# irvingzhang0512/tf_eager_object_detection

Measured on AMD Instinct MI355X. Metric: images/sec, higher is better.
Workload: dtype f32

## Files before the change

### tf_eager_object_detection_amd/csrc/nms.hip

```cpp
#include <stddef.h>
#include <string.h>

#include <algorithm>
#include <mutex>

#include "conv_diag.h"

#define NMS_CHUNK 4096
#define NMS_SEL_MAX (2 * NMS_CHUNK)
#define NMS_WORDS (NMS_CHUNK / 64)
#define SEL_BINS 4096
#define SEL_REPL 8
#define SEL_BLOCK 256
#define SEL_ITEMS 8
#define SEL_TILE (SEL_BLOCK * SEL_ITEMS)
#define PREP_ITEMS 2
#define PREP_TILE (256 * PREP_ITEMS)

typedef unsigned long long u64;

#define SCAN_LDS_BLOCKS 24
#define SCAN_LDS_CAND (SCAN_LDS_BLOCKS * 64)
#define SCAN_LDS_WORDS (SCAN_LDS_BLOCKS * (SCAN_LDS_BLOCKS - 1) / 2 * 64)
#define SCAN_LDS_SLACK_WORDS (8 * 64)
#define SCAN_DYN_LDS ((SCAN_LDS_WORDS + SCAN_LDS_SLACK_WORDS) * 8)
#define SCAN_MAT_OFF(cb, nblk) (64 * ((cb) * ((nblk)-1) - (cb) * ((cb)-1) / 2))

struct NmsState {
  int32_t n_invalid;
  int32_t kept;
  int32_t pos;
  int32_t done;
  int32_t chunk_m;
  int32_t sel_count;
  int32_t reserved0;
  int32_t sel_b1;
  uint32_t sel_below1;
  int32_t sel_b2;
  int32_t sel_overflow;
  uint32_t sel_below;
  int32_t pad[4];
};

#define SEL_COARSE 64
struct NmsHeader {
  NmsState st;
  int32_t n_invalid_acc;
  int32_t pad_acc[15];
  uint32_t hist0[SEL_REPL][SEL_COARSE];
  uint32_t hist1[SEL_REPL][SEL_BINS];
  uint32_t hist2[SEL_BINS];
  uint32_t hist3[256];
};

enum { PREP_NMS = 0, PREP_RP = 1, PREP_FPN = 2, PREP_FRCNN = 3 };

struct PrepParams {
  int n;
  PerImg<const float4*> boxes_in;
  PerImg<const float*> deltas;
  PerImg<const float*> scores;
  PerImg<const float2*> logits;
  Vec4 means, stds;
  float wmax, hmax;
  PerImg<float4*> boxes_out;
  PerImg<uint32_t*> keys;
  PerImg<NmsHeader*> hdr;
  FpnAnchorParams fpn;
};

__global__ void __launch_bounds__(256) k_zero_headers(PerImg<NmsHeader*> hdr_) {
  uint4* d = reinterpret_cast<uint4*>(hdr_.v[blockIdx.y]);
  const int i = blockIdx.x * 256 + threadIdx.x;
  if (i < (int)(sizeof(NmsHeader) / 16)) d[i] = make_uint4(0, 0, 0, 0);
}

template <int MODE>
__device__ __forceinline__ float4 d_prep_box(const PrepParams& p, int img, int e) {
  if (MODE == PREP_NMS) return p.boxes_in.v[img][e];
  float4 a;
  if (MODE == PREP_FPN) {
    a = d_fpn_anchor(p.fpn, e);
  } else if (MODE == PREP_FRCNN) {
    const int ai = e % p.fpn.A, cell = e / p.fpn.A;
    const int x = cell % p.fpn.fw[0], y = cell / p.fpn.fw[0];
    const float sx = (float)(x * p.fpn.stride[0]), sy = (float)(y * p.fpn.stride[0]);
    a = make_float4(p.fpn.wh[ai * 4 + 0] + sx, p.fpn.wh[ai * 4 + 1] + sy, p.fpn.wh[ai * 4 + 2] + sx,
                    p.fpn.wh[ai * 4 + 3] + sy);
  } else {
    a = p.boxes_in.v[img][e];
  }
  const float4 d = reinterpret_cast<const float4*>(p.deltas.v[img])[e];
  const float d0 = d.x * p.stds.v[0] + p.means.v[0];
  const float d1 = d.y * p.stds.v[1] + p.means.v[1];
  const float d2 = d.z * p.stds.v[2] + p.means.v[2];
  const float d3 = d.w * p.stds.v[3] + p.means.v[3];
  float4 b = d_decode_box(a, d0, d1, d2, d3);
  return d_clip_box(b, 0.0f, p.wmax, p.hmax);
}

__device__ __forceinline__ float4 d_candidate_box(const PrepParams& p, int mode, int img, int e) {
  switch (mode) {
    case PREP_NMS: return d_prep_box<PREP_NMS>(p, img, e);
    case PREP_RP: return d_prep_box<PREP_RP>(p, img, e);
    case PREP_FRCNN: return d_prep_box<PREP_FRCNN>(p, img, e);
    default: return d_prep_box<PREP_FPN>(p, img, e);
  }
}

struct PrepItems {
  float sc[PREP_ITEMS];
  float2 lg[PREP_ITEMS];
};

template <int MODE>
__device__ __forceinline__ void d_prep_load(const PrepParams& p, const float* __restrict__ in_scores,
                                            const float2* __restrict__ in_logits, int tile, PrepItems* v) {
#pragma unroll
  for (int it = 0; it < PREP_ITEMS; ++it) {
    const int e = tile * PREP_TILE + it * 256 + threadIdx.x;
    const int ee = e < p.n ? e : 0;
    if (MODE == PREP_FPN) {
      v->lg[it] = in_logits[ee];
    } else if (MODE == PREP_FRCNN) {
      const int loc = ee / p.fpn.A, a = ee - loc * p.fpn.A;
      const float* row = reinterpret_cast<const float*>(in_logits) + (size_t)loc * 2 * p.fpn.A;
      v->lg[it] = make_float2(row[a], row[p.fpn.A + a]);
    } else {
      v->sc[it] = in_scores[ee];
    }
  }
}

__device__ __forceinline__ uint32_t d_row16_sum(uint32_t v) {
  v += (uint32_t)__builtin_amdgcn_update_dpp(0, (int)v, 0xB1, 0xF, 0xF, false);
  v += (uint32_t)__builtin_amdgcn_update_dpp(0, (int)v, 0x4E, 0xF, 0xF, false);
  v += (uint32_t)__builtin_amdgcn_update_dpp(0, (int)v, 0x141, 0xF, 0xF, false);
  v += (uint32_t)__builtin_amdgcn_update_dpp(0, (int)v, 0x140, 0xF, 0xF, false);
  return v;
}

template <int MODE, int T>
__global__ void __launch_bounds__(256) k_rp_prepare(PrepParams p) {
  const int img = blockIdx.y;
  const float* __restrict__ in_scores = p.scores.v[img];
  const float2* __restrict__ in_logits = p.logits.v[img];
  uint32_t* __restrict__ out_keys = p.keys.v[img];
  NmsHeader* hdr = p.hdr.v[img];
  __shared__ __attribute__((aligned(16))) uint32_t h[SEL_BINS];
  uint4* h4 = reinterpret_cast<uint4*>(h);
#pragma unroll
  for (int q = 0; q < SEL_BINS / 4 / 256; ++q) h4[q * 256 + threadIdx.x] = make_uint4(0, 0, 0, 0);
  PrepItems cur;
  d_prep_load<MODE>(p, in_scores, in_logits, blockIdx.x * T, &cur);
  __syncthreads();
  int invalid = 0;
#pragma unroll
  for (int t = 0; t < T; ++t) {
    const int tile = blockIdx.x * T + t;
    PrepItems nxt;
    if (t + 1 < T) d_prep_load<MODE>(p, in_scores, in_logits, tile + 1, &nxt);
#pragma unroll
    for (int it = 0; it < PREP_ITEMS; ++it) {
      const int e = tile * PREP_TILE + it * 256 + threadIdx.x;
      if (e < p.n) {
        float s;
        if (MODE == PREP_FPN || MODE == PREP_FRCNN) s = d_fg_prob(cur.lg[it].x, cur.lg[it].y);
        else s = cur.sc[it];
        const bool valid = s > -3.402823466e+38f;
        const uint32_t k = valid ? ~d_float_asc_key(s) : 0xFFFFFFFFu;
        out_keys[e] = k;
        invalid += valid ? 0 : 1;
        atomicAdd(&h[k >> 20], 1u);
      }
    }
    if (t + 1 < T) cur = nxt;
  }
  __syncthreads();
  const int repl = blockIdx.x % SEL_REPL;
  const int lane = threadIdx.x & 63;
#pragma unroll
  for (int q = 0; q < SEL_BINS / 4 / 256; ++q) {
    const int k4 = q * 256 + threadIdx.x;
    const uint4 c = h4[k4];
    uint32_t s = c.x + c.y + c.z + c.w;
    if (__ballot(s != 0)) {
      const int first = (k4 - lane) * 4;
#pragma unroll
      for (int i = 0; i < 4; ++i) {
        const uint32_t v = h[first + i * 64 + lane];
        if (v) atomicAdd(&hdr->hist1[repl][first + i * 64 + lane], v);
      }
    }
    s = d_row16_sum(s);
    if ((threadIdx.x & 15) == 0 && s) atomicAdd(&hdr->hist0[repl][k4 >> 4], s);
  }
  if (invalid) atomicAdd(&hdr->n_invalid_acc, invalid);
}

template <int REPL>
__device__ __forceinline__ void sel_find(const uint32_t* __restrict__ hist, uint32_t target, uint32_t* result,
                                         int* lds17) {
  uint32_t v[16];
#pragma unroll
  for (int q = 0; q < 16; ++q) v[q] = 0;
#pragma unroll
  for (int r = 0; r < REPL; ++r) {
    const uint4* h4 = reinterpret_cast<const uint4*>(hist + (size_t)r * SEL_BINS) + threadIdx.x * 4;
#pragma unroll
    for (int q = 0; q < 4; ++q) {
      const uint4 t = h4[q];
      v[q * 4 + 0] += t.x; v[q * 4 + 1] += t.y; v[q * 4 + 2] += t.z; v[q * 4 + 3] += t.w;
    }
  }
  uint32_t s = 0;
#pragma unroll
  for (int q = 0; q < 16; ++q) s += v[q];
  int total;
  const uint32_t excl = (uint32_t)block_excl_scan((int)s, lds17, &total);
  if ((uint32_t)total < target) target = (uint32_t)total;
  if (threadIdx.x == 0 && total == 0) { result[0] = SEL_BINS - 1; result[1] = 0; result[2] = 0; }
  if (s > 0 && excl < target && target <= excl + s) {
    uint32_t run = excl;
#pragma unroll
    for (int q = 0; q < 16; ++q) {
      if (run < target && target <= run + v[q]) {
        result[0] = threadIdx.x * 16 + q; result[1] = run; result[2] = v[q];
      }
      run += v[q];
    }
  }
  __syncthreads();
}

__device__ __forceinline__ void sel_find1_coarse(const NmsHeader* hdr, uint32_t target, uint32_t* res) {
  if (threadIdx.x < 64) {
    const int t = threadIdx.x;
    int c = 0;
#pragma unroll
    for (int r = 0; r < SEL_REPL; ++r) c += (int)hdr->hist0[r][t];
    const int inc = wave_incl_scan(c);
    const int total = __shfl(inc, 63);
    if (total == 0) {
      if (t == 0) { res[0] = SEL_BINS - 1; res[1] = 0; }
    } else {
      const int tgt = (int)(target > (uint32_t)total ? (uint32_t)total : target);
      const u64 hitc = __ballot(c > 0 && inc - c < tgt && tgt <= inc);
      const int cb = __builtin_ctzll(hitc);
      const int below_c = __shfl(inc - c, cb);
      int v = 0;
#pragma unroll
      for (int r = 0; r < SEL_REPL; ++r) v += (int)hdr->hist1[r][cb * 64 + t];
      const int inc2 = wave_incl_scan(v);
      const u64 hitf = __ballot(v > 0 && below_c + inc2 - v < tgt && tgt <= below_c + inc2);
      const int fb = __builtin_ctzll(hitf);
      const int below_f = __shfl(inc2 - v, fb);
      if (t == 0) { res[0] = (uint32_t)(cb * 64 + fb); res[1] = (uint32_t)(below_c + below_f); }
    }
  }
  __syncthreads();
}

__global__ void __launch_bounds__(SEL_BLOCK) k_sel_hist2(PerImg<NmsHeader*> hdr_, PerImg<const uint32_t*> keys_, int n,
                                                         uint32_t target) {
  NmsHeader* hdr = hdr_.v[blockIdx.y];
  const uint32_t* __restrict__ keys = keys_.v[blockIdx.y];
  __shared__ uint32_t h[SEL_BINS];
  __shared__ uint32_t res[2];
  uint32_t key[SEL_ITEMS];
#pragma unroll
  for (int it = 0; it < SEL_ITEMS; ++it) {
    const int e = blockIdx.x * SEL_TILE + it * SEL_BLOCK + threadIdx.x;
    key[it] = (e < n) ? keys[e] : 0u;
  }
  sel_find1_coarse(hdr, target, res);
  const uint32_t b1 = res[0];
  if (blockIdx.x == 0 && threadIdx.x == 0) {
    NmsState z;
    memset(&z, 0, sizeof(z));
    z.n_invalid = hdr->n_invalid_acc;
    z.sel_b1 = (int32_t)b1; z.sel_below1 = res[1];
    hdr->st = z;
    hdr->n_invalid_acc = 0;
  }
  bool match = false;
#pragma unroll
  for (int it = 0; it < SEL_ITEMS; ++it) {
    const int e = blockIdx.x * SEL_TILE + it * SEL_BLOCK + threadIdx.x;
    match = match || (e < n && (key[it] >> 20) == b1);
  }
  if (!__syncthreads_or(match ? 1 : 0)) return;
  for (int k = threadIdx.x; k < SEL_BINS; k += SEL_BLOCK) h[k] = 0;
  __syncthreads();
#pragma unroll
  for (int it = 0; it < SEL_ITEMS; ++it) {
    const int e = blockIdx.x * SEL_TILE + it * SEL_BLOCK + threadIdx.x;
    if (e < n && (key[it] >> 20) == b1) atomicAdd(&h[(key[it] >> 8) & 0xFFFu], 1u);
  }
  __syncthreads();
  for (int k = threadIdx.x; k < SEL_BINS; k += SEL_BLOCK) {
    const uint32_t c = h[k];
    if (c) atomicAdd(&hdr->hist2[k], c);
  }
}

__global__ void __launch_bounds__(SEL_BLOCK) k_sel_compact(PerImg<NmsHeader*> hdr_, PerImg<const uint32_t*> keys_, int n,
                                                           uint32_t target, uint32_t limit, PerImg<u64*> cand_) {
  NmsHeader* hdr = hdr_.v[blockIdx.y];
  const uint32_t* __restrict__ keys = keys_.v[blockIdx.y];
  u64* __restrict__ cand = cand_.v[blockIdx.y];
  __shared__ uint32_t res[3];
  __shared__ int lds17[17];
  const uint32_t b1 = (uint32_t)hdr->st.sel_b1;
  const uint32_t below1 = hdr->st.sel_below1;
  {
    static_assert(offsetof(NmsHeader, hist1) == offsetof(NmsHeader, hist0) + sizeof(uint32_t) * SEL_REPL * SEL_COARSE, "layout");
    uint4* z = reinterpret_cast<uint4*>(&hdr->hist0[0][0]);
    for (int i = blockIdx.x * SEL_BLOCK + threadIdx.x; i < SEL_REPL * (SEL_COARSE + SEL_BINS) / 4; i += gridDim.x * SEL_BLOCK)
      z[i] = make_uint4(0, 0, 0, 0);
  }
  uint32_t total_n = (uint32_t)n;
  uint32_t t2 = (target > total_n ? total_n : target) - below1;
  sel_find<1>(hdr->hist2, t2, res, lds17);
  const uint32_t b2 = res[0];
  const bool incl = (below1 + res[1] + res[2]) <= limit;
  if (blockIdx.x == 0 && threadIdx.x == 0) {
    hdr->st.sel_b2 = (int32_t)b2;
    hdr->st.sel_overflow = incl ? 0 : 1;
    hdr->st.sel_below = below1 + res[1];
  }
  __shared__ u64 stage[SEL_TILE];
  __shared__ int s_cnt, s_base;
  if (threadIdx.x == 0) s_cnt = 0;
  uint32_t key[SEL_ITEMS];
#pragma unroll
  for (int it = 0; it < SEL_ITEMS; ++it) {
    const int e = blockIdx.x * SEL_TILE + it * SEL_BLOCK + threadIdx.x;
    key[it] = (e < n) ? keys[e] : 0xFFFFFFFFu;
  }
  __syncthreads();
  const int lane = threadIdx.x & 63;
  const u64 lt_mask = (lane == 0) ? 0ull : (~0ull >> (64 - lane));
#pragma unroll
  for (int it = 0; it < SEL_ITEMS; ++it) {
    const int e = blockIdx.x * SEL_TILE + it * SEL_BLOCK + threadIdx.x;
    const uint32_t k = key[it];
    const uint32_t p1 = k >> 20, p2 = (k >> 8) & 0xFFFu;
    const bool sel = (e < n) && (p1 < b1 || (p1 == b1 && (p2 < b2 || (incl && p2 == b2))));
    const u64 bal = __ballot(sel);
    if (bal) {
      int base = 0;
      if (lane == __builtin_ctzll(bal)) base = atomicAdd(&s_cnt, (int)__popcll(bal));
      base = __shfl(base, __builtin_ctzll(bal));
      if (sel) stage[base + (int)__popcll(bal & lt_mask)] = ((u64)k << 32) | (uint32_t)e;
    }
  }
  __syncthreads();
  const int c = s_cnt;
  if (c == 0) return;
  if (threadIdx.x == 0) s_base = atomicAdd(&hdr->st.sel_count, c);
  __syncthreads();
  const int gb = s_base;
  for (int i = threadIdx.x; i < c; i += SEL_BLOCK)
    if (gb + i < NMS_SEL_MAX) cand[gb + i] = stage[i];
}

__global__ void __launch_bounds__(SEL_BLOCK) k_sel_tie_hist(PerImg<NmsHeader*> hdr_, PerImg<const uint32_t*> keys_, int n,
                                                            PerImg<unsigned short*> bh_) {
  NmsHeader* hdr = hdr_.v[blockIdx.y];
  if (!hdr->st.sel_overflow) return;
  const uint32_t* __restrict__ keys = keys_.v[blockIdx.y];
  unsigned short* __restrict__ bh = bh_.v[blockIdx.y] + (size_t)blockIdx.x * 256;
  __shared__ uint32_t h[256];
  const uint32_t pref = ((uint32_t)hdr->st.sel_b1 << 12) | (uint32_t)hdr->st.sel_b2;
  h[threadIdx.x] = 0;
  __syncthreads();
#pragma unroll
  for (int it = 0; it < SEL_ITEMS; ++it) {
    const int e = blockIdx.x * SEL_TILE + it * SEL_BLOCK + threadIdx.x;
    if (e < n) {
      const uint32_t k = keys[e];
      if ((k >> 8) == pref) atomicAdd(&h[k & 0xFFu], 1u);
    }
  }
  __syncthreads();
  const uint32_t c = h[threadIdx.x];
  bh[threadIdx.x] = (unsigned short)c;
  if (c) atomicAdd(&hdr->hist3[threadIdx.x], c);
}

__global__ void __launch_bounds__(SEL_BLOCK) k_sel_tie_take(PerImg<NmsHeader*> hdr_, PerImg<const uint32_t*> keys_, int n,
                                                            uint32_t limit, PerImg<const unsigned short*> bh_,
                                                            PerImg<u64*> cand_) {
  NmsHeader* hdr = hdr_.v[blockIdx.y];
  if (!hdr->st.sel_overflow) return;
  const uint32_t below = hdr->st.sel_below;
  if (below >= limit) return;
  const uint32_t quota = limit - below;
  const uint32_t* __restrict__ keys = keys_.v[blockIdx.y];
  const unsigned short* __restrict__ bh = bh_.v[blockIdx.y];
  u64* __restrict__ cand = cand_.v[blockIdx.y];
  __shared__ int lds17[17];
  __shared__ uint32_t s_b3, s_q3, s_pre;
  __shared__ int s_wave[4];
  __shared__ u64 stage[SEL_TILE];
  __shared__ int s_cnt, s_base;
  const uint32_t pref = ((uint32_t)hdr->st.sel_b1 << 12) | (uint32_t)hdr->st.sel_b2;
  const uint32_t hv = hdr->hist3[threadIdx.x];
  int total;
  const uint32_t excl = (uint32_t)block_excl_scan((int)hv, lds17, &total);
  if (threadIdx.x == 0) { s_b3 = 256; s_q3 = 0; s_pre = 0; s_cnt = 0; }
  __syncthreads();
  if (hv > 0 && excl < quota && quota <= excl + hv) { s_b3 = threadIdx.x; s_q3 = quota - excl; }
  __syncthreads();
  const uint32_t b3 = s_b3, q3 = s_q3;
  if (b3 < 256) {
    uint32_t mine = 0;
    for (int b = threadIdx.x; b < (int)blockIdx.x; b += SEL_BLOCK) mine += bh[(size_t)b * 256 + b3];
    int tot2;
    block_excl_scan((int)mine, lds17, &tot2);
    if (threadIdx.x == 0) s_pre = (uint32_t)tot2;
  }
  __syncthreads();
  uint32_t run = s_pre;
  const int lane = threadIdx.x & 63, wv = threadIdx.x >> 6;
  const u64 lt_mask = (lane == 0) ? 0ull : (~0ull >> (64 - lane));
  for (int it = 0; it < SEL_ITEMS; ++it) {
    const int e = blockIdx.x * SEL_TILE + it * SEL_BLOCK + threadIdx.x;
    const uint32_t k = (e < n) ? keys[e] : 0xFFFFFFFFu;
    const bool inbin = (e < n) && (k >> 8) == pref;
    const uint32_t v = k & 0xFFu;
    const bool tie = inbin && v == b3;
    const u64 tb = __ballot(tie);
    if (lane == 0) s_wave[wv] = (int)__popcll(tb);
    __syncthreads();
    uint32_t before = run;
    for (int q = 0; q < wv; ++q) before += (uint32_t)s_wave[q];
    const uint32_t my_rank = before + (uint32_t)__popcll(tb & lt_mask);
    const uint32_t all4 = (uint32_t)(s_wave[0] + s_wave[1] + s_wave[2] + s_wave[3]);
    const bool sel = inbin && (v < b3 || (tie && my_rank < q3));
    const u64 bal = __ballot(sel);
    if (bal) {
      int base = 0;
      if (lane == __builtin_ctzll(bal)) base = atomicAdd(&s_cnt, (int)__popcll(bal));
      base = __shfl(base, __builtin_ctzll(bal));
      if (sel) stage[base + (int)__popcll(bal & lt_mask)] = ((u64)k << 32) | (uint32_t)e;
    }
    run += all4;
    __syncthreads();
  }
  const int c = s_cnt;
  if (c == 0) return;
  if (threadIdx.x == 0) s_base = atomicAdd(&hdr->st.sel_count, c);
  __syncthreads();
  const int gb = s_base;
  for (int i = threadIdx.x; i < c; i += SEL_BLOCK)
    if (gb + i < NMS_SEL_MAX) cand[gb + i] = stage[i];
}

#define RANK_THREADS 1024
__global__ void __launch_bounds__(RANK_THREADS) k_sel_rank(PerImg<NmsHeader*> hdr_, int n, int cap0, PerImg<const u64*> cand_,
                                                          PrepParams prep, int mode, PerImg<uint32_t*> sel_idx_,
                                                          PerImg<float4*> sboxes_, PerImg<float4*> sorig_) {
  NmsHeader* hdr = hdr_.v[blockIdx.y];
  const u64* __restrict__ cand = cand_.v[blockIdx.y];
  uint32_t* __restrict__ sel_idx = sel_idx_.v[blockIdx.y];
  float4* __restrict__ sboxes = sboxes_.v[blockIdx.y];
  float4* __restrict__ sorig = sorig_.v[blockIdx.y];
  __shared__ u64 all[NMS_CHUNK];
  __shared__ int part[16][64];
  NmsState* st = &hdr->st;
  const int cnt = min(st->sel_count, NMS_SEL_MAX);
  if (blockIdx.x == 0 && threadIdx.x == 0) st->chunk_m = min(min(cnt, cap0), n - st->n_invalid);
  if (blockIdx.x == 0) {
    uint4* z = reinterpret_cast<uint4*>(hdr->hist2);
    for (int i = threadIdx.x; i < SEL_BINS / 4; i += RANK_THREADS) z[i] = make_uint4(0, 0, 0, 0);
    if (threadIdx.x < 256) hdr->hist3[threadIdx.x] = 0;
  }
  if (blockIdx.x * 64 >= cnt) return;
  const int lane = threadIdx.x & 63, w = threadIdx.x >> 6;
  const int i = blockIdx.x * 64 + lane;
  const u64 mine = (i < cnt) ? cand[i] : ~0ull;
  float4 bx = make_float4(0.0f, 0.0f, 0.0f, 0.0f);
  if (w == 0 && i < cnt) bx = d_candidate_box(prep, mode, blockIdx.y, (int)(uint32_t)mine);
  int c = 0;
  for (int t0 = 0; t0 < cnt; t0 += NMS_CHUNK) {
    const int tc = min(NMS_CHUNK, cnt - t0);
    __syncthreads();
    for (int k = threadIdx.x; k < tc; k += RANK_THREADS) all[k] = cand[t0 + k];
    __syncthreads();
    const int per = (tc + 15) >> 4;
    const int lo = w * per, hi = min(tc, lo + per);
    for (int j = lo; j < hi; ++j) c += (all[j] < mine) ? 1 : 0;
  }
  part[w][lane] = c;
  __syncthreads();
  if (w == 0 && i < cnt) {
    int r = 0;
#pragma unroll
    for (int k = 0; k < 16; ++k) r += part[k][lane];
    const uint32_t idx = (uint32_t)mine;
    sel_idx[r] = idx;
    if (r < cap0) {
      sboxes[r] = d_norm_box(bx);
      sorig[r] = bx;
    }
  }
}

__global__ void __launch_bounds__(256) k_nms_gather(PerImg<NmsState*> st_, int n, int cap, int from_sel,
                                                    PrepParams prep, int mode, PerImg<const uint32_t*> sorted_idx_,
                                                    PerImg<float4*> sboxes_, PerImg<float4*> sorig_) {
  NmsState* st = st_.v[blockIdx.y];
  const uint32_t* __restrict__ sorted_idx = sorted_idx_.v[blockIdx.y];
  float4* __restrict__ sboxes = sboxes_.v[blockIdx.y];
  float4* __restrict__ sorig = sorig_.v[blockIdx.y];
  const int pos = st->pos, nv = n - st->n_invalid;
  const int lim = from_sel ? min(nv, min(st->sel_count, NMS_SEL_MAX)) : nv;
  const int m = st->done ? 0 : max(0, min(cap, lim - pos));
  const int i = blockIdx.x * 256 + threadIdx.x;
  if (i == 0) st->chunk_m = m;
  if (i < m) {
    const float4 bx = d_candidate_box(prep, mode, blockIdx.y, (int)sorted_idx[pos + i]);
    sboxes[i] = d_norm_box(bx);
    sorig[i] = bx;
  }
}

__global__ void __launch_bounds__(256) k_nms_cross(PerImg<const NmsState*> st_, PerImg<const float4*> sboxes_,
                                                   PerImg<const float4*> kept_boxes_, float thr,
                                                   PerImg<u64*> removed_init_) {
  const NmsState* st = st_.v[blockIdx.y];
  const float4* __restrict__ sboxes = sboxes_.v[blockIdx.y];
  const float4* __restrict__ kept_boxes = kept_boxes_.v[blockIdx.y];
  u64* __restrict__ removed_init = removed_init_.v[blockIdx.y];
  __shared__ float4 kb[256];
  __shared__ float ka[256];
  const int m = st->chunk_m, nk = st->kept;
  if (blockIdx.x * 256 >= m) return;
  const int j = blockIdx.x * 256 + threadIdx.x;
  const float4 b = (j < m) ? sboxes[j] : make_float4(0, 0, 0, 0);
  const float area = d_box_area(b);
  bool sup = false;
  for (int k0 = 0; k0 < nk; k0 += 256) {
    __syncthreads();
    if (k0 + threadIdx.x < nk) {
      float4 t = kept_boxes[k0 + threadIdx.x];
      kb[threadIdx.x] = t;
      ka[threadIdx.x] = d_box_area(t);
    }
    __syncthreads();
    const int lim = min(256, nk - k0);
    for (int k = 0; k < lim; ++k) sup = sup || d_iou_gt(b, area, kb[k], ka[k], thr);
  }
  u64 bal = __ballot(sup && j < m);
  if ((threadIdx.x & 63) == 0) removed_init[j >> 6] = bal;
}

__global__ void __launch_bounds__(256) k_nms_mask(PerImg<const NmsState*> st_, PerImg<const float4*> sboxes_, float thr,
                                                  PerImg<u64*> Lt_, PerImg<u64*> diag_, int packed) {
// ... 459 lines not shown
          const int l = olvl ? min(max(olvl[r], 0), nlo - 1) : 0;
          int qy, qx;
          bkt[e] = d_roi_order_bucket(osrc[r], l, sp.ord_inv_h, sp.ord_inv_w, &qy, &qx);
          slot[e] = atomicAdd(&ocnt[bkt[e]], 1);
        } else if (r < K) {
          order[r] = r;
        }
      }
      __syncthreads();
      scan_order_buckets(ocnt, nb, keptpre);
      __syncthreads();
#pragma unroll
      for (int e = 0; e < 2; ++e)
        if (bkt[e] >= 0) order[ocnt[bkt[e]] + slot[e]] = tid + e * SCAN_THREADS;
    } else {
      if (tid < K) order[tid] = tid;
      if (tid + SCAN_THREADS < K) order[tid + SCAN_THREADS] = tid + SCAN_THREADS;
    }
  }
}

struct NmsWorkspace {
  NmsHeader* hdr;
  uint32_t *keys_a, *vals_a, *keys_b, *vals_b, *hist;
  u64* cand;
  float4 *sboxes, *sorig, *kept_boxes;
  u64 *Lt, *diag, *removed_init;
};

static size_t nms_carve(int n, int max_out, void* ws, size_t ws_bytes, NmsWorkspace* o) {
  OdetArena ar{(char*)ws, ws ? ws_bytes : (size_t)-1, 0};
  size_t nn = (size_t)(n > 0 ? n : 1);
  size_t kk = (size_t)(max_out > 0 ? max_out : 1);
#define TAKE(field, T, count)                                 \
  do {                                                        \
    T* p_ = ar.take<T>(count);                                \
    if (o) o->field = ws ? p_ : nullptr;                      \
  } while (0)
  TAKE(hdr, NmsHeader, 1);
  TAKE(keys_a, uint32_t, nn);
  TAKE(vals_a, uint32_t, nn);
  TAKE(keys_b, uint32_t, nn);
  TAKE(vals_b, uint32_t, std::max(nn, (size_t)NMS_SEL_MAX));
  TAKE(hist, uint32_t, odet_sort_hist_entries(n));
  TAKE(cand, u64, NMS_SEL_MAX);
  TAKE(sboxes, float4, NMS_CHUNK);
  TAKE(sorig, float4, NMS_CHUNK);
  TAKE(kept_boxes, float4, kk);
  TAKE(Lt, u64, (size_t)NMS_WORDS * NMS_CHUNK);
  TAKE(diag, u64, NMS_CHUNK);
  TAKE(removed_init, u64, NMS_WORDS);
#undef TAKE
  return ar.off + 256;
}

extern "C" size_t odet_nms_workspace_bytes(int n, int max_output) {
  return nms_carve(n, max_output, nullptr, 0, nullptr);
}

static int first_chunk_target(int n, int K, int first_chunk) {
  long long c = ((long long)K * 3 / 2 + 63) / 64 * 64;
  if (c > 64) c -= 32;
  if (first_chunk > 0) c = std::max<long long>(c, ((long long)first_chunk + 63) / 64 * 64 - 32);
  if (c < 256) c = 256;
  if (c > NMS_CHUNK) c = NMS_CHUNK;
  if (c > n) c = n;
  return (int)c;
}

static inline int tri_tiles(int cap) {
  int nb = (cap + 63) / 64;
  return nb * (nb + 1) / 2;
}

struct NmsPlan {
  int n, K, first_chunk, B, sync_free;
  int blind;
  int target;
  int lds0, limit;
  int wide;
  int sel_target, sel_limit;
  int prep_grid, sel_grid, rank_wgs;
  int prep_tiles;
  int cap0, tiles0;
  int cap, tiles;
  int further;
  int sel_chunks;
  int full_sort;
  int fail_empty_chunk;
  int max_chunks;
};

#define PREP_RESIDENT_WGS 2048
#define PREP_MAX_TILES 4
static int nms_prep_tiles(int prep_grid, int B) {
  for (int t = 1; t < PREP_MAX_TILES; t *= 2)
    if ((long long)((prep_grid + t - 1) / t) * B <= PREP_RESIDENT_WGS) return t;
  return PREP_MAX_TILES;
}

static int nms_plan(int n, int K, int first_chunk, int blind_chunks, int sync_free, int B, NmsPlan* out) {
  NmsPlan p;
  p.n = n; p.K = K; p.first_chunk = first_chunk; p.B = B; p.sync_free = sync_free ? 1 : 0;
  p.blind = blind_chunks < 1 ? 1 : blind_chunks;
  p.target = first_chunk_target(n, K, first_chunk);
  p.lds0 = p.target <= SCAN_LDS_CAND ? 1 : 0;
  p.limit = p.lds0 ? SCAN_LDS_CAND : NMS_CHUNK;
  p.wide = (p.sync_free && p.blind >= 2) ? 1 : 0;
  p.sel_target = p.wide ? (int)std::min<long long>(n, (long long)p.target + NMS_CHUNK) : p.target;
  p.sel_limit = p.wide ? NMS_SEL_MAX : p.limit;
  p.prep_grid = (n + PREP_TILE - 1) / PREP_TILE;
  p.prep_tiles = nms_prep_tiles(p.prep_grid, B);
  p.sel_grid = (n + SEL_TILE - 1) / SEL_TILE;
  if (p.wide)
    ODET_REQUIRE((size_t)p.sel_grid * 256 * sizeof(unsigned short) <= (size_t)NMS_WORDS * NMS_CHUNK * sizeof(u64),
                 "odet_nms: %d anchors exceed the tie split's scratch (the bit-matrix buffer)", n);
  p.rank_wgs = (std::min(n, p.sel_limit) + 63) / 64;
  p.cap0 = std::min(p.limit, (n + 63) / 64 * 64);
  p.tiles0 = tri_tiles(p.cap0);
  p.cap = std::min(NMS_CHUNK, (n + 63) / 64 * 64);
  p.tiles = tri_tiles(p.cap);
  p.further = p.sync_free ? p.blind - 1 : 0;
  p.sel_chunks = p.further >= 1 ? 1 : 0;
  p.full_sort = p.further >= 2 ? 1 : 0;
  p.fail_empty_chunk = p.sync_free ? p.blind - 1 : -1;
  p.max_chunks = p.sync_free ? 0 : (n + NMS_CHUNK - 1) / NMS_CHUNK + 1;
  *out = p;
  return ODET_OK;
}

#ifdef ODET_DIAG
static std::mutex g_nms_plan_mutex;
static odet_debug_nms_plan_t g_last_nms_plan;
static void nms_plan_to_record(const NmsPlan& p, odet_debug_nms_plan_t* r, long long count) {
  *r = odet_debug_nms_plan_t{p.n, p.K, p.first_chunk, p.B, p.sync_free, p.blind, p.target, p.lds0, p.limit, p.wide,
                             p.sel_target, p.sel_limit, p.prep_grid, p.sel_grid, p.rank_wgs, p.cap0, p.tiles0, p.cap,
                             p.tiles, p.further, p.sel_chunks, p.full_sort, p.fail_empty_chunk, p.max_chunks, count};
}
static void nms_diag_record(const NmsPlan& p) {
  std::lock_guard<std::mutex> lock(g_nms_plan_mutex);
  nms_plan_to_record(p, &g_last_nms_plan, g_last_nms_plan.count + 1);
}
extern "C" int odet_debug_last_nms_plan(odet_debug_nms_plan_t* out) {
  ODET_REQUIRE(out, "odet_debug_last_nms_plan: null record");
  std::lock_guard<std::mutex> lock(g_nms_plan_mutex);
  *out = g_last_nms_plan;
  return ODET_OK;
}
extern "C" int odet_debug_nms_plan(int n, int K, int first_chunk, int blind_chunks, int sync_free, int B,
                                   odet_debug_nms_plan_t* out) {
  ODET_REQUIRE(out && n > 0 && K > 0 && first_chunk >= 0 && first_chunk <= NMS_CHUNK && B >= 1 && B <= ODET_MAX_BATCH &&
               (sync_free || B == 1), "odet_debug_nms_plan: bad arguments");
  NmsPlan p;
  const int rc = nms_plan(n, K, first_chunk, blind_chunks, sync_free, B, &p);
  if (rc == ODET_OK) nms_plan_to_record(p, out, 0);
  return rc;
}
#define ODET_DIAG_NMS_PLAN(plan)               \
  do {                                         \
    nms_diag_record(plan);                     \
    if (odet_diag_plan_only()) return ODET_OK; \
  } while (0)
#define ODET_DIAG_NMS_TRIVIAL()                \
  do {                                         \
    if (odet_diag_plan_only()) return ODET_OK; \
  } while (0)
#else
#define ODET_DIAG_NMS_PLAN(plan) \
  do {                           \
  } while (0)
#define ODET_DIAG_NMS_TRIVIAL() \
  do {                          \
  } while (0)
#endif

struct NmsImage {
  const float4* boxes_in;
  const float* deltas;
  const float* scores;
  const float2* logits;
  float4* boxes_out;
  const float4* boxes;
  int32_t* out_idx;
  float* out_boxes;
  int32_t* out_count;
  int32_t* out_done;
  AssignOut assign;
  void* ws;
  size_t ws_bytes;
};

struct NmsJob {
  int mode;
  PrepParams prep;
  int n, K;
  float thr;
// ... 37 lines not shown
  else if (J.mode == PREP_FRCNN) nms_prepare_launch<PREP_FRCNN>(J, P, st);
  else nms_prepare_launch<PREP_FPN>(J, P, st);
  ODET_LAUNCH_CHECK();
  return ODET_OK;
}

struct NmsChunks {
  const NmsJob& J;
  const NmsPlan& P;
  hipStream_t st;
  ScanParams sp;
  PerImg<const NmsState*> cstates;
  PerImg<float4*> sboxes, sorig;
  PerImg<const float4*> csboxes, kept;
  PerImg<u64*> Lt, diag, rinit;

  int launch(int from_sel, const PerImg<const uint32_t*>& sorted_idx, int fail_empty) const {
    const dim3 rows((P.cap + 255) / 256, P.B), block(256);
    hipLaunchKernelGGL(k_nms_gather, rows, block, 0, st, sp.st, P.n, P.cap, from_sel, J.prep, J.mode, sorted_idx, sboxes, sorig);
    ODET_LAUNCH_CHECK();
    hipLaunchKernelGGL(k_nms_cross, rows, block, 0, st, cstates, csboxes, kept, J.thr, rinit);
    ODET_LAUNCH_CHECK();
    hipLaunchKernelGGL(k_nms_mask, dim3(P.tiles, P.B), block, 0, st, cstates, csboxes, J.thr, Lt, diag, 0);
    ODET_LAUNCH_CHECK();
    ScanParams s = sp;
    s.use_init = 1; s.sorted_idx = sorted_idx; s.fail_empty = fail_empty;
    hipLaunchKernelGGL(HIP_KERNEL_NAME(k_nms_scan<false>), dim3(1, P.B), dim3(SCAN_THREADS), scan_order_lds(s), st, s);
    ODET_LAUNCH_CHECK();
    return ODET_OK;
  }
};

static int nms_done_on_host(const NmsState* state, hipStream_t st, bool* done) {
  NmsState h;
  ODET_HIP(hipMemcpyAsync(&h, state, sizeof(h), hipMemcpyDeviceToHost, st));
  ODET_HIP(hipStreamSynchronize(st));
  *done = h.done != 0;
  return ODET_OK;
}

static int nms_run(NmsJob& J, hipStream_t st) {
  const int n = J.n, K = J.K, B = J.B;
  if (B < 1 || B > ODET_MAX_BATCH) return odet_set_error(ODET_E_INVALID, "odet_nms: batch %d out of range", B);
  NmsWorkspace w[ODET_MAX_BATCH];
  const size_t need = nms_carve(n, K, nullptr, 0, nullptr);
  for (int i = 0; i < B; ++i) {
    if (!J.img[i].ws || J.img[i].ws_bytes < need)
      return odet_set_error(ODET_E_WORKSPACE, "odet_nms: workspace too small (%zu < %zu)", J.img[i].ws_bytes, need);
    nms_carve(n, K, J.img[i].ws, J.img[i].ws_bytes, &w[i]);
  }
  if (B > 1) {
    for (int i = 0; i < B; ++i)
      if (!J.img[i].out_done)
        return odet_set_error(ODET_E_INVALID, "odet_nms: batches need the sync-free mode (out_done)");
  }
  NmsPlan P;
  const int prc = nms_plan(n, K, J.first_chunk, J.blind_chunks, J.img[0].out_done != nullptr, B, &P);
  if (prc != ODET_OK) return prc;
  ODET_DIAG_NMS_PLAN(P);
  int rc = nms_scan_setup();
  if (rc != ODET_OK) return rc;
  const PerImg<NmsHeader*> hdrs = per_img<NmsHeader*>(J, [&](int i) { return w[i].hdr; });
  const PerImg<const uint32_t*> keys = per_img<const uint32_t*>(J, [&](int i) { return (const uint32_t*)w[i].keys_a; });
  if (!J.ws_clean) {
    hipLaunchKernelGGL(k_zero_headers, dim3((unsigned)((sizeof(NmsHeader) / 16 + 255) / 256), B), dim3(256), 0, st, hdrs);
    ODET_LAUNCH_CHECK();
  }
  J.prep.n = n;
  J.prep.boxes_in = per_img<const float4*>(J, [&](int i) { return J.img[i].boxes_in; });
  J.prep.deltas = per_img<const float*>(J, [&](int i) { return J.img[i].deltas; });
  J.prep.scores = per_img<const float*>(J, [&](int i) { return J.img[i].scores; });
  J.prep.logits = per_img<const float2*>(J, [&](int i) { return J.img[i].logits; });
  J.prep.boxes_out = per_img<float4*>(J, [&](int i) { return J.img[i].boxes_out; });
  J.prep.keys = per_img<uint32_t*>(J, [&](int i) { return w[i].keys_a; });
  J.prep.hdr = hdrs;
  rc = nms_prepare(J, P, st);
  if (rc != ODET_OK) return rc;
  const uint32_t sel_target = (uint32_t)P.sel_target;
  NmsChunks ch{J, P, st};
  ch.sboxes = per_img<float4*>(J, [&](int i) { return w[i].sboxes; });
  ch.sorig = per_img<float4*>(J, [&](int i) { return w[i].sorig; });
  {
    dim3 grid(P.sel_grid, B), block(SEL_BLOCK);
    hipLaunchKernelGGL(k_sel_hist2, grid, block, 0, st, hdrs, keys, n, sel_target);
    ODET_LAUNCH_CHECK();
    const PerImg<u64*> cand = per_img<u64*>(J, [&](int i) { return w[i].cand; });
    hipLaunchKernelGGL(k_sel_compact, grid, block, 0, st, hdrs, keys, n, sel_target, (uint32_t)P.sel_limit, cand);
    ODET_LAUNCH_CHECK();
    if (P.wide) {
      const PerImg<unsigned short*> bh = per_img<unsigned short*>(J, [&](int i) { return (unsigned short*)w[i].Lt; });
      hipLaunchKernelGGL(k_sel_tie_hist, grid, block, 0, st, hdrs, keys, n, bh);
      ODET_LAUNCH_CHECK();
      hipLaunchKernelGGL(k_sel_tie_take, grid, block, 0, st, hdrs, keys, n, sel_target,
                         per_img<const unsigned short*>(J, [&](int i) { return (const unsigned short*)w[i].Lt; }), cand);
      ODET_LAUNCH_CHECK();
    }
    hipLaunchKernelGGL(k_sel_rank, dim3(P.rank_wgs, B), dim3(RANK_THREADS), 0, st, hdrs, n, P.limit,
                       per_img<const u64*>(J, [&](int i) { return (const u64*)w[i].cand; }), J.prep, J.mode,
                       per_img<uint32_t*>(J, [&](int i) { return w[i].vals_b; }), ch.sboxes, ch.sorig);
    ODET_LAUNCH_CHECK();
  }
  ch.cstates = per_img<const NmsState*>(J, [&](int i) { return (const NmsState*)&w[i].hdr->st; });
  ch.csboxes = per_img<const float4*>(J, [&](int i) { return (const float4*)w[i].sboxes; });
  ch.kept = per_img<const float4*>(J, [&](int i) { return (const float4*)w[i].kept_boxes; });
  ch.Lt = per_img<u64*>(J, [&](int i) { return w[i].Lt; });
  ch.diag = per_img<u64*>(J, [&](int i) { return w[i].diag; });
  ch.rinit = per_img<u64*>(J, [&](int i) { return w[i].removed_init; });
  const PerImg<const uint32_t*> ranked = per_img<const uint32_t*>(J, [&](int i) { return (const uint32_t*)w[i].vals_b; });
  ScanParams& sp = ch.sp;
  sp.st = per_img<NmsState*>(J, [&](int i) { return &w[i].hdr->st; });
  sp.Lt = per_img<const u64*>(J, [&](int i) { return (const u64*)w[i].Lt; });
  sp.diag_up = per_img<const u64*>(J, [&](int i) { return (const u64*)w[i].diag; });
  sp.removed_init = per_img<const u64*>(J, [&](int i) { return (const u64*)w[i].removed_init; });
  sp.sboxes = ch.csboxes;
  sp.sorig = per_img<const float4*>(J, [&](int i) { return (const float4*)w[i].sorig; });
  sp.sorted_idx = ranked;
  sp.out_idx = per_img<int32_t*>(J, [&](int i) { return J.img[i].out_idx; });
  sp.out_boxes = per_img<float4*>(J, [&](int i) { return (float4*)J.img[i].out_boxes; });
  sp.kept_boxes = per_img<float4*>(J, [&](int i) { return w[i].kept_boxes; });
  sp.out_count = per_img<int32_t*>(J, [&](int i) { return J.img[i].out_count; });
  sp.out_done = per_img<int32_t*>(J, [&](int i) { return J.img[i].out_done; });
  sp.as_rois = per_img<float4*>(J, [&](int i) { return J.img[i].assign.rois; });
  sp.as_level = per_img<int32_t*>(J, [&](int i) { return J.img[i].assign.level; });
  sp.as_perm = per_img<int64_t*>(J, [&](int i) { return J.img[i].assign.perm; });
  sp.as_counts = per_img<int32_t*>(J, [&](int i) { return J.img[i].assign.counts; });
  sp.as_order = per_img<int32_t*>(J, [&](int i) { return K <= ODET_FUSED_ORDER_MAX_ROIS ? J.img[i].assign.order : nullptr; });
  sp.ord_inv_h = 1.0f / (J.prep.hmax + 1.0f); sp.ord_inv_w = 1.0f / (J.prep.wmax + 1.0f);
  sp.n = n; sp.use_init = 0; sp.K = K;
  auto fail_empty = [&](int c) { return (J.fail_empty && c == P.fail_empty_chunk) ? 1 : 0; };
  sp.fail_empty = fail_empty(0);
  sp.min_level = J.img[0].assign.min_level; sp.max_level = J.img[0].assign.max_level;
  hipLaunchKernelGGL(k_nms_mask, dim3(P.tiles0, B), dim3(256), 0, st, ch.cstates, ch.csboxes, J.thr, ch.Lt, ch.diag, P.lds0);
  ODET_LAUNCH_CHECK();
  if (P.lds0)
    hipLaunchKernelGGL(HIP_KERNEL_NAME(k_nms_scan<true>), dim3(1, B), dim3(SCAN_THREADS), SCAN_DYN_LDS, st, sp);
  else
    hipLaunchKernelGGL(HIP_KERNEL_NAME(k_nms_scan<false>), dim3(1, B), dim3(SCAN_THREADS), scan_order_lds(sp), st, sp);
  ODET_LAUNCH_CHECK();
  if (P.sync_free) {
    for (int c = 1; c <= P.sel_chunks && rc == ODET_OK; ++c) rc = ch.launch(1, ranked, fail_empty(c));
    if (rc != ODET_OK || !P.full_sort) return rc;
    OdetSortImage si[ODET_MAX_BATCH];
    for (int i = 0; i < B; ++i)
      si[i] = OdetSortImage{w[i].keys_a, w[i].vals_a, w[i].keys_b, w[i].vals_b, w[i].hist, &w[i].hdr->st.done};
    rc = odet_sort_keys_desc_batch(n, B, si, st);
    const PerImg<const uint32_t*> order = per_img<const uint32_t*>(J, [&](int i) { return (const uint32_t*)w[i].vals_a; });
    for (int c = P.sel_chunks + 1; c <= P.further && rc == ODET_OK; ++c) rc = ch.launch(0, order, fail_empty(c));
    return rc;
  }
  const NmsState* state = &w[0].hdr->st;
  bool done = false;
  if (P.blind == 1) {
    rc = nms_done_on_host(state, st, &done);
    if (rc != ODET_OK || done) return rc;
  }
  uint32_t* sorted = nullptr;
  rc = odet_sort_keys_desc(n, w[0].keys_a, w[0].vals_a, w[0].keys_b, w[0].vals_b, w[0].hist, &w[0].hdr->st.done, &sorted, st);
  const PerImg<const uint32_t*> order = per_img<const uint32_t*>(J, [&](int) { return (const uint32_t*)sorted; });
  for (int c = 1; c <= P.max_chunks && rc == ODET_OK; ++c) {
    if (c >= P.blind && !(c == 1 && P.blind == 1)) {
      rc = nms_done_on_host(state, st, &done);
      if (rc != ODET_OK || done) break;
    }
    rc = ch.launch(0, order, 0);
  }
  return rc;
}

static int nms_trivial(int32_t* out_count, int32_t* out_done, hipStream_t st) {
  ODET_DIAG_NMS_TRIVIAL();
  ODET_HIP(hipMemsetAsync(out_count, 0, sizeof(int32_t), st));
// ... 232 lines not shown
```

Before: 29670.

## Split radix selection into single key pass plus boundary-bucket filter

```diff
diff --git a/tf_eager_object_detection_amd/csrc/nms.hip b/tf_eager_object_detection_amd/csrc/nms.hip
--- a/tf_eager_object_detection_amd/csrc/nms.hip
+++ b/tf_eager_object_detection_amd/csrc/nms.hip
@@ -46,7 +46,8 @@
 struct NmsHeader {
   NmsState st;
   int32_t n_invalid_acc;
-  int32_t pad_acc[15];
+  uint32_t bnd_count;
+  int32_t pad_acc[14];
   uint32_t hist0[SEL_REPL][SEL_COARSE];
   uint32_t hist1[SEL_REPL][SEL_BINS];
   uint32_t hist2[SEL_BINS];
@@ -196,6 +197,7 @@
     if ((threadIdx.x & 15) == 0 && s) atomicAdd(&hdr->hist0[repl][k4 >> 4], s);
   }
   if (invalid) atomicAdd(&hdr->n_invalid_acc, invalid);
+  if (blockIdx.x == 0 && threadIdx.x == 0) hdr->st.sel_count = 0;
 }
 
 template <int REPL>
@@ -261,108 +263,170 @@
   __syncthreads();
 }
 
-__global__ void __launch_bounds__(SEL_BLOCK) k_sel_hist2(PerImg<NmsHeader*> hdr_, PerImg<const uint32_t*> keys_, int n,
-                                                         uint32_t target) {
-  NmsHeader* hdr = hdr_.v[blockIdx.y];
-  const uint32_t* __restrict__ keys = keys_.v[blockIdx.y];
-  __shared__ uint32_t h[SEL_BINS];
-  __shared__ uint32_t res[2];
-  uint32_t key[SEL_ITEMS];
-#pragma unroll
-  for (int it = 0; it < SEL_ITEMS; ++it) {
-    const int e = blockIdx.x * SEL_TILE + it * SEL_BLOCK + threadIdx.x;
-    key[it] = (e < n) ? keys[e] : 0u;
-  }
-  sel_find1_coarse(hdr, target, res);
-  const uint32_t b1 = res[0];
-  if (blockIdx.x == 0 && threadIdx.x == 0) {
-    NmsState z;
-    memset(&z, 0, sizeof(z));
-    z.n_invalid = hdr->n_invalid_acc;
-    z.sel_b1 = (int32_t)b1; z.sel_below1 = res[1];
-    hdr->st = z;
-    hdr->n_invalid_acc = 0;
-  }
-  bool match = false;
-#pragma unroll
-  for (int it = 0; it < SEL_ITEMS; ++it) {
-    const int e = blockIdx.x * SEL_TILE + it * SEL_BLOCK + threadIdx.x;
-    match = match || (e < n && (key[it] >> 20) == b1);
-  }
-  if (!__syncthreads_or(match ? 1 : 0)) return;
-  for (int k = threadIdx.x; k < SEL_BINS; k += SEL_BLOCK) h[k] = 0;
-  __syncthreads();
-#pragma unroll
-  for (int it = 0; it < SEL_ITEMS; ++it) {
-    const int e = blockIdx.x * SEL_TILE + it * SEL_BLOCK + threadIdx.x;
-    if (e < n && (key[it] >> 20) == b1) atomicAdd(&h[(key[it] >> 8) & 0xFFFu], 1u);
-  }
-  __syncthreads();
-  for (int k = threadIdx.x; k < SEL_BINS; k += SEL_BLOCK) {
-    const uint32_t c = h[k];
-    if (c) atomicAdd(&hdr->hist2[k], c);
-  }
-}
-
-__global__ void __launch_bounds__(SEL_BLOCK) k_sel_compact(PerImg<NmsHeader*> hdr_, PerImg<const uint32_t*> keys_, int n,
-                                                           uint32_t target, uint32_t limit, PerImg<u64*> cand_) {
+template <int T>
+__global__ void __launch_bounds__(SEL_BLOCK) k_sel_split(PerImg<NmsHeader*> hdr_, PerImg<const uint32_t*> keys_, int n,
+                                                         uint32_t target, PerImg<u64*> cand_, PerImg<u64*> bnd_) {
   NmsHeader* hdr = hdr_.v[blockIdx.y];
   const uint32_t* __restrict__ keys = keys_.v[blockIdx.y];
   u64* __restrict__ cand = cand_.v[blockIdx.y];
-  __shared__ uint32_t res[3];
-  __shared__ int lds17[17];
-  const uint32_t b1 = (uint32_t)hdr->st.sel_b1;
-  const uint32_t below1 = hdr->st.sel_below1;
+  u64* __restrict__ bnd = bnd_.v[blockIdx.y];
+  __shared__ __attribute__((aligned(16))) uint32_t h[SEL_BINS];
+  __shared__ uint32_t res[2];
+  __shared__ int s_wc[SEL_BLOCK / 64][2];
+  __shared__ int s_base[2];
+  const int tid = threadIdx.x, lane = tid & 63, wv = tid >> 6;
+  const u64 lt_mask = (lane == 0) ? 0ull : (~0ull >> (64 - lane));
+  const int e0 = blockIdx.x * (T * SEL_TILE) + tid;
+  uint32_t key[T * SEL_ITEMS];
+#pragma unroll
+  for (int q = 0; q < T * SEL_ITEMS; ++q) {
+    const int e = e0 + q * SEL_BLOCK;
+    key[q] = (e < n) ? keys[e] : 0xFFFFFFFFu;
+  }
+  sel_find1_coarse(hdr, target, res);
+  const uint32_t b1 = res[0], below1 = res[1];
+  if (blockIdx.x == 0 && tid == 0) {
+    NmsState* s = &hdr->st;
+    s->n_invalid = hdr->n_invalid_acc;
+    s->kept = 0; s->pos = 0; s->done = 0; s->chunk_m = 0; s->reserved0 = 0;
+    s->sel_b1 = (int32_t)b1; s->sel_below1 = below1;
+    s->sel_b2 = 0; s->sel_overflow = 0; s->sel_below = 0;
+    s->pad[0] = 0; s->pad[1] = 0; s->pad[2] = 0; s->pad[3] = 0;
+    hdr->n_invalid_acc = 0;
+  }
+  int ca = 0, cb = 0;
+#pragma unroll
+  for (int q = 0; q < T * SEL_ITEMS; ++q) {
+    const bool in = e0 + q * SEL_BLOCK < n;
+    const uint32_t p1 = key[q] >> 20;
+    ca += (int)__popcll(__ballot(in && p1 < b1));
+    cb += (int)__popcll(__ballot(in && p1 == b1));
+  }
+  if (lane == 0) { s_wc[wv][0] = ca; s_wc[wv][1] = cb; }
+  __syncthreads();
+  int tot_a = 0, tot_b = 0, off_a = 0, off_b = 0;
+#pragma unroll
+  for (int w = 0; w < SEL_BLOCK / 64; ++w) {
+    if (w == wv) { off_a = tot_a; off_b = tot_b; }
+    tot_a += s_wc[w][0]; tot_b += s_wc[w][1];
+  }
+  if (!(tot_a | tot_b)) return;
+  if (tid < 2) {
+    const int c = tid ? tot_b : tot_a;
+    s_base[tid] = c ? (tid ? (int)atomicAdd(&hdr->bnd_count, (uint32_t)c) : atomicAdd(&hdr->st.sel_count, c)) : 0;
+  }
+  if (tot_b) {
+    uint4* h4 = reinterpret_cast<uint4*>(h);
+#pragma unroll
+    for (int q = 0; q < SEL_BINS / 4 / SEL_BLOCK; ++q) h4[q * SEL_BLOCK + tid] = make_uint4(0, 0, 0, 0);
+  }
+  __syncthreads();
+  off_a += s_base[0]; off_b += s_base[1];
+#pragma unroll
+  for (int q = 0; q < T * SEL_ITEMS; ++q) {
+    const int e = e0 + q * SEL_BLOCK;
+    const bool in = e < n;
+    const uint32_t k = key[q], p1 = k >> 20;
+    const bool sa = in && p1 < b1, sb = in && p1 == b1;
+    const u64 ba = __ballot(sa), bb = __ballot(sb);
+    const u64 pair = ((u64)k << 32) | (uint32_t)e;
+    if (sa) {
+      const int at = off_a + (int)__popcll(ba & lt_mask);
+      if (at < NMS_SEL_MAX) cand[at] = pair;
+    }
+    if (sb) {
+      const int at = off_b + (int)__popcll(bb & lt_mask);
+      if (at < n) bnd[at] = pair;
+      atomicAdd(&h[(k >> 8) & 0xFFFu], 1u);
+    }
+    off_a += (int)__popcll(ba); off_b += (int)__popcll(bb);
+  }
+  if (!tot_b) return;
+  __syncthreads();
+  const uint4* h4 = reinterpret_cast<const uint4*>(h);
+#pragma unroll
+  for (int q = 0; q < SEL_BINS / 4 / SEL_BLOCK; ++q) {
+    const int k4 = q * SEL_BLOCK + tid;
+    const uint4 c = h4[k4];
+    if (c.x) atomicAdd(&hdr->hist2[k4 * 4 + 0], c.x);
+    if (c.y) atomicAdd(&hdr->hist2[k4 * 4 + 1], c.y);
+    if (c.z) atomicAdd(&hdr->hist2[k4 * 4 + 2], c.z);
+    if (c.w) atomicAdd(&hdr->hist2[k4 * 4 + 3], c.w);
+  }
+}
+
+__global__ void __launch_bounds__(SEL_BLOCK) k_sel_filter(PerImg<NmsHeader*> hdr_, int n, uint32_t target, uint32_t limit,
+                                                          PerImg<u64*> cand_, PerImg<const u64*> bnd_) {
+  NmsHeader* hdr = hdr_.v[blockIdx.y];
   {
     static_assert(offsetof(NmsHeader, hist1) == offsetof(NmsHeader, hist0) + sizeof(uint32_t) * SEL_REPL * SEL_COARSE, "layout");
     uint4* z = reinterpret_cast<uint4*>(&hdr->hist0[0][0]);
     for (int i = blockIdx.x * SEL_BLOCK + threadIdx.x; i < SEL_REPL * (SEL_COARSE + SEL_BINS) / 4; i += gridDim.x * SEL_BLOCK)
       z[i] = make_uint4(0, 0, 0, 0);
   }
-  uint32_t total_n = (uint32_t)n;
-  uint32_t t2 = (target > total_n ? total_n : target) - below1;
+  const int nb = min((int)hdr->bnd_count, n);
+  if ((int)blockIdx.x * SEL_TILE >= nb) return;
+  u64* __restrict__ cand = cand_.v[blockIdx.y];
+  const ulonglong2* __restrict__ bl2 = reinterpret_cast<const ulonglong2*>(bnd_.v[blockIdx.y]);
+  __shared__ uint32_t res[3];
+  __shared__ int lds17[17];
+  __shared__ int s_wc[SEL_BLOCK / 64];
+  __shared__ int s_base;
+  const int tid = threadIdx.x, lane = tid & 63, wv = tid >> 6;
+  const u64 lt_mask = (lane == 0) ? 0ull : (~0ull >> (64 - lane));
+  const int nb2 = (nb + 1) / 2;
+  ulonglong2 pr[SEL_ITEMS / 2];
+#pragma unroll
+  for (int u = 0; u < SEL_ITEMS / 2; ++u) {
+    const int i2 = (int)blockIdx.x * (SEL_TILE / 2) + u * SEL_BLOCK + tid;
+    pr[u] = (i2 < nb2) ? bl2[i2] : make_ulonglong2(~0ull, ~0ull);
+  }
+  const uint32_t below1 = hdr->st.sel_below1;
+  const uint32_t total_n = (uint32_t)n;
+  const uint32_t t2 = (target > total_n ? total_n : target) - below1;
   sel_find<1>(hdr->hist2, t2, res, lds17);
   const uint32_t b2 = res[0];
   const bool incl = (below1 + res[1] + res[2]) <= limit;
-  if (blockIdx.x == 0 && threadIdx.x == 0) {
+  if (blockIdx.x == 0 && tid == 0) {
     hdr->st.sel_b2 = (int32_t)b2;
     hdr->st.sel_overflow = incl ? 0 : 1;
     hdr->st.sel_below = below1 + res[1];
   }
-  __shared__ u64 stage[SEL_TILE];
-  __shared__ int s_cnt, s_base;
-  if (threadIdx.x == 0) s_cnt = 0;
-  uint32_t key[SEL_ITEMS];
-#pragma unroll
-  for (int it = 0; it < SEL_ITEMS; ++it) {
-    const int e = blockIdx.x * SEL_TILE + it * SEL_BLOCK + threadIdx.x;
-    key[it] = (e < n) ? keys[e] : 0xFFFFFFFFu;
-  }
-  __syncthreads();
-  const int lane = threadIdx.x & 63;
-  const u64 lt_mask = (lane == 0) ? 0ull : (~0ull >> (64 - lane));
-#pragma unroll
-  for (int it = 0; it < SEL_ITEMS; ++it) {
-    const int e = blockIdx.x * SEL_TILE + it * SEL_BLOCK + threadIdx.x;
-    const uint32_t k = key[it];
-    const uint32_t p1 = k >> 20, p2 = (k >> 8) & 0xFFFu;
-    const bool sel = (e < n) && (p1 < b1 || (p1 == b1 && (p2 < b2 || (incl && p2 == b2))));
-    const u64 bal = __ballot(sel);
-    if (bal) {
-      int base = 0;
-      if (lane == __builtin_ctzll(bal)) base = atomicAdd(&s_cnt, (int)__popcll(bal));
-      base = __shfl(base, __builtin_ctzll(bal));
-      if (sel) stage[base + (int)__popcll(bal & lt_mask)] = ((u64)k << 32) | (uint32_t)e;
-    }
-  }
-  __syncthreads();
-  const int c = s_cnt;
-  if (c == 0) return;
-  if (threadIdx.x == 0) s_base = atomicAdd(&hdr->st.sel_count, c);
-  __syncthreads();
-  const int gb = s_base;
-  for (int i = threadIdx.x; i < c; i += SEL_BLOCK)
-    if (gb + i < NMS_SEL_MAX) cand[gb + i] = stage[i];
+  const uint32_t p2_end = b2 + (incl ? 1u : 0u);
+  u64 bal[SEL_ITEMS];
+  int cnt = 0;
+#pragma unroll
+  for (int u = 0; u < SEL_ITEMS / 2; ++u) {
+    const int i = 2 * ((int)blockIdx.x * (SEL_TILE / 2) + u * SEL_BLOCK + tid);
+    bal[2 * u] = __ballot(i < nb && (uint32_t)((pr[u].x >> 40) & 0xFFFu) < p2_end);
+    bal[2 * u + 1] = __ballot(i + 1 < nb && (uint32_t)((pr[u].y >> 40) & 0xFFFu) < p2_end);
+    cnt += (int)__popcll(bal[2 * u]) + (int)__popcll(bal[2 * u + 1]);
+  }
+  if (lane == 0) s_wc[wv] = cnt;
+  __syncthreads();
+  int tot = 0, at = 0;
+#pragma unroll
+  for (int w = 0; w < SEL_BLOCK / 64; ++w) {
+    if (w == wv) at = tot;
+    tot += s_wc[w];
+  }
+  if (!tot) return;
+  if (tid == 0) s_base = atomicAdd(&hdr->st.sel_count, tot);
+  __syncthreads();
+  at += s_base;
+#pragma unroll
+  for (int u = 0; u < SEL_ITEMS / 2; ++u) {
+    if ((bal[2 * u] >> lane) & 1) {
+      const int o = at + (int)__popcll(bal[2 * u] & lt_mask);
+      if (o < NMS_SEL_MAX) cand[o] = pr[u].x;
+    }
+    at += (int)__popcll(bal[2 * u]);
+    if ((bal[2 * u + 1] >> lane) & 1) {
+      const int o = at + (int)__popcll(bal[2 * u + 1] & lt_mask);
+      if (o < NMS_SEL_MAX) cand[o] = pr[u].y;
+    }
+    at += (int)__popcll(bal[2 * u + 1]);
+  }
 }
 
 __global__ void __launch_bounds__(SEL_BLOCK) k_sel_tie_hist(PerImg<NmsHeader*> hdr_, PerImg<const uint32_t*> keys_, int n,
@@ -476,6 +540,7 @@
     uint4* z = reinterpret_cast<uint4*>(hdr->hist2);
     for (int i = threadIdx.x; i < SEL_BINS / 4; i += RANK_THREADS) z[i] = make_uint4(0, 0, 0, 0);
     if (threadIdx.x < 256) hdr->hist3[threadIdx.x] = 0;
+    if (threadIdx.x == 0) hdr->bnd_count = 0;
   }
   if (blockIdx.x * 64 >= cnt) return;
   const int lane = threadIdx.x & 63, w = threadIdx.x >> 6;
@@ -1101,6 +1166,7 @@
   int sel_target, sel_limit;
   int prep_grid, sel_grid, rank_wgs;
   int prep_tiles;
+  int sel_tiles;
   int cap0, tiles0;
   int cap, tiles;
   int further;
@@ -1116,6 +1182,12 @@
   for (int t = 1; t < PREP_MAX_TILES; t *= 2)
     if ((long long)((prep_grid + t - 1) / t) * B <= PREP_RESIDENT_WGS) return t;
   return PREP_MAX_TILES;
+}
+
+#define SEL_ONE_ROUND_WGS 256
+#define SEL_MAX_TILES 2
+static int nms_sel_tiles(int sel_grid, int B) {
+  return (long long)sel_grid * B <= SEL_ONE_ROUND_WGS ? 1 : SEL_MAX_TILES;
 }
 
 static int nms_plan(int n, int K, int first_chunk, int blind_chunks, int sync_free, int B, NmsPlan* out) {
@@ -1131,6 +1203,7 @@
   p.prep_grid = (n + PREP_TILE - 1) / PREP_TILE;
   p.prep_tiles = nms_prep_tiles(p.prep_grid, B);
   p.sel_grid = (n + SEL_TILE - 1) / SEL_TILE;
+  p.sel_tiles = nms_sel_tiles(p.sel_grid, B);
   if (p.wide)
     ODET_REQUIRE((size_t)p.sel_grid * 256 * sizeof(unsigned short) <= (size_t)NMS_WORDS * NMS_CHUNK * sizeof(u64),
                  "odet_nms: %d anchors exceed the tie split's scratch (the bit-matrix buffer)", n);
@@ -1334,11 +1407,23 @@
   ch.sorig = per_img<float4*>(J, [&](int i) { return w[i].sorig; });
   {
     dim3 grid(P.sel_grid, B), block(SEL_BLOCK);
-    hipLaunchKernelGGL(k_sel_hist2, grid, block, 0, st, hdrs, keys, n, sel_target);
-    ODET_LAUNCH_CHECK();
     const PerImg<u64*> cand = per_img<u64*>(J, [&](int i) { return w[i].cand; });
-    hipLaunchKernelGGL(k_sel_compact, grid, block, 0, st, hdrs, keys, n, sel_target, (uint32_t)P.sel_limit, cand);
-    ODET_LAUNCH_CHECK();
+    {
+      const PerImg<u64*> bnd = per_img<u64*>(J, [&](int i) {
+        return (size_t)((char*)(w[i].keys_b + n) - (char*)w[i].vals_a) >= (size_t)n * sizeof(u64) ? (u64*)w[i].vals_a : nullptr;
+      });
+      for (int i = 0; i < B; ++i)
+        if (!bnd.v[i]) return odet_set_error(ODET_E_WORKSPACE, "odet_nms: the sort buffers do not hold the boundary list");
+      const dim3 sgrid((P.sel_grid + P.sel_tiles - 1) / P.sel_tiles, B);
+      if (P.sel_tiles == 1)
+        hipLaunchKernelGGL(HIP_KERNEL_NAME(k_sel_split<1>), sgrid, block, 0, st, hdrs, keys, n, sel_target, cand, bnd);
+      else
+        hipLaunchKernelGGL(HIP_KERNEL_NAME(k_sel_split<SEL_MAX_TILES>), sgrid, block, 0, st, hdrs, keys, n, sel_target, cand, bnd);
+      ODET_LAUNCH_CHECK();
+      hipLaunchKernelGGL(k_sel_filter, grid, block, 0, st, hdrs, n, sel_target, (uint32_t)P.sel_limit, cand,
+                         per_img<const u64*>(J, [&](int i) { return (const u64*)bnd.v[i]; }));
+      ODET_LAUNCH_CHECK();
+    }
     if (P.wide) {
       const PerImg<unsigned short*> bh = per_img<unsigned short*>(J, [&](int i) { return (unsigned short*)w[i].Lt; });
       hipLaunchKernelGGL(k_sel_tie_hist, grid, block, 0, st, hdrs, keys, n, bh);
```

After: 29910, median of 6. About the same (+0.8%).
